# openai/multiagent-particle-envs

Hardware: AMD Instinct MI355X
Metric: env steps/sec (whole node), simple_spread N=3, batch=65536 per GPU (higher is better)
Workload: dtype f32; 1 GPU; simple_spread A=3 L=3, 65536 worlds/GPU, fresh one-hot moves, reset every 25 steps; steps commanded to the step server; protocol=fresh, step-server (one doorbell per episode), batch_per_gpu=65536, global_batch=65536, mode=step-server, commands=auto, barrier_backend=none

## Files before the change

### multiagent_particle_envs_amd/csrc/mpe_split.hip

```cpp
#include <type_traits>

#include "mpe_internal.h"

#ifndef MPE_SPLIT_ABLATE
#define MPE_SPLIT_ABLATE 0
#endif

#ifdef MPE_PHASE_CLOCK
#define MPE_STAMP(k)                                                                                              \
  do {                                                                                                            \
    if (blockIdx.x < 4 && lane == 0 && b.force && t < 32)                                                         \
      reinterpret_cast<unsigned long long *>(b.force)[(((size_t)blockIdx.x * 16 + role) * 32 + t) * 8 + (k)] =     \
          __builtin_amdgcn_s_memtime();                                                                           \
  } while (0)
#else
#define MPE_STAMP(k) do { } while (0)
#endif

#ifdef MPE_DEVICE_SPAN
#define MPE_SPAN_BEGIN() const unsigned long long span_t0_ = (unsigned long long)wall_clock64()
#define MPE_SPAN_END()                                                                                             \
  do {                                                                                                             \
    if (b_in.force && (threadIdx.x & 63) == 0 && (threadIdx.x >> 6) < 8) {                                           \
      const uintptr_t sp_ = reinterpret_cast<uintptr_t>(b_in.force);                                                \
      if (sp_ & 1) asm volatile("s_waitcnt vmcnt(0) lgkmcnt(0)" ::: "memory");                                      \
      ulonglong2 st_;                                                                                              \
      st_.x = span_t0_;                                                                                            \
      st_.y = (unsigned long long)wall_clock64();                                                                  \
      reinterpret_cast<ulonglong2 *>(sp_ & ~(uintptr_t)7)[(size_t)blockIdx.x * 8 + (threadIdx.x >> 6)] = st_;       \
    }                                                                                                              \
  } while (0)
#else
#define MPE_SPAN_BEGIN() do { } while (0)
#define MPE_SPAN_END() do { } while (0)
#endif

namespace mpe {

#ifndef MPE_SPLIT_DUAL
#define MPE_SPLIT_DUAL 1
#endif
#ifndef MPE_SPLIT_DUAL_OWN_DRAW
#define MPE_SPLIT_DUAL_OWN_DRAW (1 << MPE_SCN_SPREAD)
#endif
template <int KIND>
constexpr bool dual_own_draw() { return ((MPE_SPLIT_DUAL_OWN_DRAW) >> KIND) & 1; }

template <int KIND>
constexpr bool dual_kind() {
  return (MPE_SPLIT_DUAL) &&
         (KIND == MPE_SCN_SIMPLE || KIND == MPE_SCN_SPREAD || KIND == MPE_SCN_TAG || KIND == MPE_SCN_ADVERSARY || KIND == MPE_SCN_PUSH);
}

template <int KIND, int A, int L, int NADV>
struct SplitShape {
  static constexpr int E = A + L;
  static constexpr int XW = KIND == MPE_SCN_SPREAD ? 4 + L
                            : (KIND == MPE_SCN_SIMPLE || KIND == MPE_SCN_ADVERSARY || KIND == MPE_SCN_PUSH ||
                               KIND == MPE_SCN_SPEAKER_LISTENER || KIND == MPE_SCN_REFERENCE) ? 5
                            : KIND == MPE_SCN_WORLD_COMM ? 6 : 4;
  static constexpr int DC = KIND == MPE_SCN_SPEAKER_LISTENER ? 3 : KIND == MPE_SCN_REFERENCE ? 10
                            : (KIND == MPE_SCN_CRYPTO || KIND == MPE_SCN_WORLD_COMM) ? 4 : 2;
  static constexpr int NCH = (KIND == MPE_SCN_ADVERSARY || KIND == MPE_SCN_PUSH || KIND == MPE_SCN_SPEAKER_LISTENER) ? 1
                             : (KIND == MPE_SCN_REFERENCE || KIND == MPE_SCN_CRYPTO) ? 2 : 0;
  static constexpr int DMAX = KIND == MPE_SCN_SIMPLE   ? 2 + 2 * L
                              : KIND == MPE_SCN_SPREAD ? 4 + 2 * L + 4 * (A - 1)
                              : KIND == MPE_SCN_TAG    ? 4 + 2 * L + 2 * (A - 1) + 2 * (A - NADV)
                              : KIND == MPE_SCN_ADVERSARY ? 2 + 2 * L + 2 * (A - 1)
                              : KIND == MPE_SCN_PUSH   ? 7 + 5 * L + 2 * (A - 1)
                              : KIND == MPE_SCN_SPEAKER_LISTENER ? 2 + 2 * L + 3
                              : KIND == MPE_SCN_REFERENCE ? 2 + 2 * L + 3 + 10
                              : KIND == MPE_SCN_CRYPTO ? 8
                              : KIND == MPE_SCN_WORLD_COMM ? 4 + 2 * L + 2 * (A - 1) + 2 * (A - NADV) + 2 + 4
// ... 399 lines not shown
};
__device__ __forceinline__ unsigned long long door_load(const unsigned long long *p) {
  const unsigned long long v = __hip_atomic_load(p, __ATOMIC_RELAXED, __HIP_MEMORY_SCOPE_SYSTEM);
  const uint32_t lo = __builtin_amdgcn_readfirstlane((uint32_t)v), hi = __builtin_amdgcn_readfirstlane((uint32_t)(v >> 32));
  return ((unsigned long long)hi << 32) | lo;
}
__device__ __forceinline__ void drain_stores() { asm volatile("s_waitcnt vmcnt(0)" ::: "memory"); }

template <int KIND, int A, int L, int NADV, bool ROLL, int RP ,
          bool DUALP = false ,
          bool SERVE = false ,
          bool POL = false >
__device__ __forceinline__ void split_body(float *const g_pos, float *const g_vel, const float *const g_act, const int32_t *const g_ids,
                                           const size_t B, const int g_wpw, const int g_observe_only, const unsigned g_movable,
                                           const NarrowDesc &d, const MpeBuffers &b_in, const RollArgs &ra, const ServeArgs &sv,
                                           const PolArgs &pol) {
  static_assert(!SERVE || (ROLL && RP == kRowsSc1), "the step server: a rollout instantiation, write-through stores");
  static_assert(!POL || (ROLL && !SERVE && !DUALP), "the policy rollout: a single-role rollout instantiation");
  static_assert(!POL || KIND == MPE_SCN_SIMPLE || KIND == MPE_SCN_SPREAD || KIND == MPE_SCN_ADVERSARY || KIND == MPE_SCN_PUSH,
                "the policy rollout: scenarios whose observation rows read no other agent's velocity");
  constexpr int WM = SERVE ? kWordRowSys : (ROLL ? kWordDrawn : kWordRow);
  using S = SplitShape<KIND, A, L, NADV>;
  MPE_SPAN_BEGIN();
  MpeBuffers b = b_in;
  b.pos = g_pos;
  b.vel = g_vel;
  b.act = g_act;
  b.ids = g_ids;
  constexpr int E = A + L, XW = S::XW;
  constexpr int AUX = SERVE ? kRowsSc1 : aux_policy<KIND, RP>();
  extern __shared__ __attribute__((aligned(16))) float smem[];
  const int lane = threadIdx.x & (kWave - 1);
  constexpr bool DUAL = DUALP && ROLL;
  constexpr bool OWN_DRAW = DUAL && dual_own_draw<KIND>();
  constexpr int NAW = DUAL ? 2 * A : A;
  const int role = __builtin_amdgcn_readfirstlane((int)(threadIdx.x >> 6));
  const bool is_agent = role < NAW;
  const bool is_rows = DUAL && role >= A && role < NAW;
  const int i = is_agent ? (role >= A ? role - A : role) : 0;
  const int wpw = g_wpw;
  const size_t w0 = (size_t)blockIdx.x * (size_t)wpw;
  if (w0 >= B) return;
#ifdef MPE_STRESS_DELAY_WAVE
  if (role == (MPE_STRESS_DELAY_WAVE) % A)
    for (int k = 0; k < 10; ++k) __builtin_amdgcn_s_sleep(127);
#endif
  const int nvalid = (B - w0) < (size_t)wpw ? (int)(B - w0) : wpw;
  const bool live = lane < nvalid;
  const unsigned ln = (unsigned)(live ? lane : nvalid - 1) & 63u;
  const size_t w = w0 + (size_t)ln;
  float *const xch = smem;
  float *const tile = smem + (ROLL ? 2 : 1) * A * XW * kWave + i * S::tile_floats(ROLL);
  int *const mv = reinterpret_cast<int *>(smem + (ROLL ? 2 : 1) * A * XW * kWave + A * S::tile_floats(ROLL));

  const int T = ROLL ? ra.T : 1;
  const size_t obs_stride = (ra.trajectory || SERVE) ? (size_t)d.obs_off[A] * B : 0;
  const size_t row_stride = (ra.trajectory || SERVE) ? (size_t)A * B : 0;
  int blk0 = 0, mvt0 = 0;
  unsigned long long seen = 0;
  int *const idle_cnt = reinterpret_cast<int *>(smem + SplitShape<KIND, A, L, NADV>::lds_bytes(true) / sizeof(float));
  if constexpr (SERVE) {
    blk0 = (int)(ra.step0 % (uint64_t)sv.slots);
    mvt0 = (int)(ra.step0 % (uint64_t)sv.ring);
    if (threadIdx.x < 3) idle_cnt[threadIdx.x] = 0;
    __syncthreads();
  }
// ... 12 lines not shown
    if (seen > g) return true;
    drain_stores();
    bool told = t == 0;
    if (!publisher && !told && lane == 0) __hip_atomic_fetch_add(&idle_cnt[t & 1], 1, __ATOMIC_RELEASE, __HIP_MEMORY_SCOPE_WORKGROUP);
    const unsigned long long t_begin = (unsigned long long)wall_clock64();
    for (;;) {
      if (publisher && !told) {
        const int n = __builtin_amdgcn_readfirstlane(__hip_atomic_load(&idle_cnt[t & 1], __ATOMIC_ACQUIRE, __HIP_MEMORY_SCOPE_WORKGROUP));
        if (n >= NAW) {
          if (lane == 0) __hip_atomic_store(sv.flag + blockIdx.x, g, __ATOMIC_RELAXED, __HIP_MEMORY_SCOPE_SYSTEM);
          told = true;
        }
      }
      __builtin_amdgcn_s_sleep(4);
      seen = door_load(sv.door);
      if (seen > g) return true;
      if ((unsigned long long)wall_clock64() - t_begin > sv.timeout_ticks) {
        if (lane == 0) {
          __hip_atomic_store(sv.status, 1u, __ATOMIC_RELAXED, __HIP_MEMORY_SCOPE_SYSTEM);
          __hip_atomic_store(&idle_cnt[2], 1, __ATOMIC_RELAXED, __HIP_MEMORY_SCOPE_WORKGROUP);
        }
        return false;
      }
    }
  };
  auto next_commanded = [&](const int t) -> bool {
    if constexpr (!SERVE) return false;
    return t + 1 < T && seen > ra.step0 + (unsigned long long)t + 1;
  };
  auto aborted = [&]() -> bool {
    if constexpr (!SERVE) return false;
    return __builtin_amdgcn_readfirstlane(__hip_atomic_load(&idle_cnt[2], __ATOMIC_RELAXED, __HIP_MEMORY_SCOPE_WORKGROUP)) != 0;
  };

  if (!is_agent) {
    constexpr bool TRACK = ROLL && (KIND == MPE_SCN_CRYPTO || KIND == MPE_SCN_WORLD_COMM);
    const uint64_t gw_r = ra.world_offset + w;
    int goal_r = (ROLL && KIND == MPE_SCN_CRYPTO) ? (b.choice + wave_off(w0))[ln] : 0;
    float food[4] = {0.f, 0.f, 0.f, 0.f};
    if (ROLL && KIND == MPE_SCN_WORLD_COMM) {
#pragma unroll
      for (int f = 0; f < 2; ++f) {
        food[2 * f] = (b.pos + wave_off((size_t)(2 * (A + 1 + f)) * B + w0))[ln];
        food[2 * f + 1] = (b.pos + wave_off((size_t)(2 * (A + 1 + f) + 1) * B + w0))[ln];
      }
    }
    float sz[E];
#pragma unroll
    for (int e = 0; e < E; ++e) sz[e] = d.size[e];
    pin_s(sz);
    int cd = -1;
    uint64_t ep_r = 0;
    if (TRACK && ra.episode_len > 0) {
      const uint64_t len = (uint64_t)ra.episode_len, r = ra.step0 % len;
      cd = r == 0 ? 0 : (int)(len - r);
      ep_r = ra.step0 / len + (r ? 1 : 0);
    }
    for (int t = 0; t < T; ++t) {
      MPE_STAMP(0);
      if (SERVE && !wait_door(t, true)) {
        __syncthreads();
        return;
      }
      if (TRACK && cd >= 0) {
        if (cd == 0) {
          if (KIND == MPE_SCN_CRYPTO) goal_r = choice_draw(ra.seed, gw_r, ep_r, 0, d.choice_pop[0]);
          if (KIND == MPE_SCN_WORLD_COMM) {
#pragma unroll
            for (int f = 0; f < 2; ++f) reset_draw(ra.seed, gw_r, ep_r, A + 1 + f, ra.landmark_range, food[2 * f], food[2 * f + 1]);
          }
          ++ep_r;
          cd = ra.episode_len - 1;
        } else {
          --cd;
        }
      }
      if (ROLL && !SERVE && !OWN_DRAW && !POL && t + 1 < T) {
        const uint64_t gt1 = ra.step0 + (uint64_t)t + 1;
#pragma unroll
        for (int q = 0; q < (A + 3) / 4; ++q) {
          const U4 o = action_block(ra.seed, gw_r, gt1, q);
          const uint32_t word[4] = {o.x, o.y, o.z, o.w};
#pragma unroll
          for (int k = 0; k < 4; ++k)
            if (4 * q + k < A) mv[(((t + 1) & 1) * A + 4 * q + k) * kWave + lane] = move_of(word[k]);
        }
      }
      const float *const X = xch + (ROLL ? (t & 1) * A * XW * kWave : 0);
      MPE_STAMP(1);
      if (SERVE) drain_stores();
      __syncthreads();
      if (SERVE) {
        if (t > 0 && lane == 0) __hip_atomic_store(sv.flag + blockIdx.x, ra.step0 + (unsigned long long)t, __ATOMIC_RELAXED, __HIP_MEMORY_SCOPE_SYSTEM);
        if (lane == 0) idle_cnt[t & 1] = 0;
        if (aborted()) return;
      }
      MPE_STAMP(2);
      if (!(MPE_SPLIT_ABLATE & 2))
      reward_wave<KIND, A, L, NADV, ROLL, AUX, WM>(d, sz, with_words(t), X, lane, live, ln, B, w0, (size_t)block_of(t) * row_stride + w0,
                                                   ra.seed, gw_r, ra.step0 + (uint64_t)t, goal_r, food);
      MPE_STAMP(3);
    }
    if (SERVE) {
      drain_stores();
      __syncthreads();
      if (lane == 0) __hip_atomic_store(sv.flag + blockIdx.x, ra.step0 + (unsigned long long)T, __ATOMIC_RELAXED, __HIP_MEMORY_SCOPE_SYSTEM);
    }
    MPE_SPAN_END();
    return;
  }

  float px[E], py[E];
#pragma unroll
  for (int e = 0; e < E; ++e) {
    px[e] = (b.pos + wave_off((size_t)(2 * e) * B + w0))[ln];
    py[e] = (b.pos + wave_off((size_t)(2 * e + 1) * B + w0))[ln];
  }
  float mvx = (b.vel + wave_off((size_t)(2 * i) * B + w0))[ln];
  float mvy = (b.vel + wave_off((size_t)(2 * i + 1) * B + w0))[ln];
  const bool movable_i = (g_movable >> i) & 1u;
  const bool step_world = ROLL || !g_observe_only;
  float ux0 = 0.f, uy0 = 0.f;
  if (!ROLL && step_world && movable_i && (b.act || b.ids)) fetch_action_wave(b, B, i, w0, ln, 1.0f, ux0, uy0);

  float kc[9 + E];
  kc[0] = d.size[i]; kc[1] = d.inv_mass[i]; kc[2] = d.accel[i]; kc[3] = d.max_speed[i];
  kc[4] = d.dt; kc[5] = d.damp; kc[6] = d.cforce; kc[7] = d.cmargin; kc[8] = d.cmargin_inv;
#pragma unroll
// ... 14 lines not shown
  constexpr int NCH = S::NCH, DC = S::DC;
  int goal = NCH >= 1 ? (b.choice + wave_off(w0))[ln] : 0;
  int pick1 = NCH >= 2 ? (b.choice + wave_off(B + w0))[ln] : 0;

  int countdown = -1;
  uint64_t ep = 0;
  if (ROLL && ra.episode_len > 0) {
    const uint64_t len = (uint64_t)ra.episode_len, r = ra.step0 % len;
    countdown = r == 0 ? 0 : (int)(len - r);
    ep = ra.step0 / len + (r ? 1 : 0);
  }

  float gx = 0.f, gy = 0.f;
  [[maybe_unused]] bool did_reset = false;
  auto roll_reset = [&]() -> bool {
    const bool reset_now = countdown == 0;
    if (countdown >= 0) countdown = reset_now ? ra.episode_len - 1 : countdown - 1;
    if (reset_now) {
#pragma unroll
      for (int e = 0; e < E; ++e) reset_draw(ra.seed, gw, ep, e, e < A ? 1.0f : ra.landmark_range, px[e], py[e]);
#pragma unroll
      for (int a = 0; a < A; ++a)
        if (a == i) { mx = px[a]; my = py[a]; }
      mvx = 0.f;
      mvy = 0.f;
      if (NCH >= 1) goal = choice_draw(ra.seed, gw, ep, 0, d.choice_pop[0]);
      if (NCH >= 2) pick1 = choice_draw(ra.seed, gw, ep, 1, d.choice_pop[1]);
      ++ep;
      if (SERVE) did_reset = true;
    }
    return reset_now;
  };
  [[maybe_unused]] float pa1 = 0.f, pa2 = 0.f, pa3 = 0.f, pa4 = 0.f;
  auto step_forces = [&](const int t, float &fx, float &fy) {
    float ux, uy;
    const uint64_t gt = ra.step0 + (uint64_t)t;
    if (ROLL) {
      if constexpr (!POL) roll_reset();
      if constexpr (SERVE) {
        const float *const mt = sv.act_ring + (size_t)((mvt0 + t) % sv.ring) * ((size_t)A * B * MPE_ACTION_DIM);
        typedef float vf4 __attribute__((ext_vector_type(4)));
        const float *const mp = mt + wave_off(((size_t)i * B + w0) * MPE_ACTION_DIM) + (ln * MPE_ACTION_DIM + 1);
        vf4 m4;
        asm volatile("global_load_dwordx4 %0, %1, off sc0 sc1\n\ts_waitcnt vmcnt(0)" : "=&v"(m4) : "v"(mp) : "memory");
        if (movable_i) {
          ux = (m4.x - m4.y) * accel_i;
          uy = (m4.z - m4.w) * accel_i;
        } else {
          ux = 0.f;
          uy = 0.f;
        }
      } else if constexpr (POL) {
        ux = (pa1 - pa2) * accel_i;
        uy = (pa3 - pa4) * accel_i;
      } else {
      const int m = (t == 0 || OWN_DRAW) ? action_draw(ra.seed, gw, gt, i) : mv[((t & 1) * A + i) * kWave + lane];
      ux = ((m == 1 ? 1.f : 0.f) - (m == 2 ? 1.f : 0.f)) * accel_i;
      uy = ((m == 3 ? 1.f : 0.f) - (m == 4 ? 1.f : 0.f)) * accel_i;
      }
    } else if (step_world && movable_i) {
      if (b.act || b.ids) { ux = ux0 * accel_i; uy = uy0 * accel_i; }
      else fetch_action_wave(b, B, i, w0, ln, accel_i, ux, uy);
    } else {
      ux = 0.f;
      uy = 0.f;
    }
    fx = ux + 0.f;
    fy = uy + 0.f;
    if (movable_i && step_world && collide_i && !(MPE_SPLIT_ABLATE & 1)) {
#pragma unroll
      for (int j = 0; j < E; ++j) {
        if (j == i) continue;
        if (!((d.collide >> j) & 1u)) continue;
        float cx, cy;
        contact_force(mx - px[j], my - py[j], size_i + size_e[j], k_cforce, k_cmargin, k_cmargin_inv, cx, cy);
        fx = cx + fx;
        fy = cy + fy;
// ... 7 lines not shown
      if (live && (!ROLL || t == T - 1)) store_state<AUX>(b, B, i, w0, ln, mx, my, mvx, mvy);
#endif
    }
#ifdef MPE_PHASE_CLOCK
    asm volatile("" ::"v"(mx), "v"(my), "v"(mvx), "v"(mvy));
#endif
  };
  auto publish = [&](const int t) {
    float *const X = xch + (ROLL ? (t & 1) * A * XW * kWave : 0);
    X[(i * XW + 0) * kWave + lane] = mx;
    X[(i * XW + 1) * kWave + lane] = my;
    X[(i * XW + 2) * kWave + lane] = mvx;
    X[(i * XW + 3) * kWave + lane] = mvy;
    if (KIND == MPE_SCN_SPREAD) {
#pragma unroll
      for (int l = 0; l < L; ++l) X[(i * XW + 4 + l) * kWave + lane] = sq2d(mx - px[A + l], my - py[A + l]);
    }
    if (KIND == MPE_SCN_SIMPLE) X[(i * XW + 4) * kWave + lane] = sq2d(mx - px[A], my - py[A]);
    if (HAS_GOAL || KIND == MPE_SCN_SPEAKER_LISTENER) {
      goal_pos<A, L>(px, py, goal, gx, gy);
      X[(i * XW + 4) * kWave + lane] = sq2d(mx - gx, my - gy);
    }
    if constexpr (KIND == MPE_SCN_REFERENCE) {
      goal_pos<A, L>(px, py, i == 0 ? pick1 : goal, gx, gy);
      X[(i * XW + 4) * kWave + lane] = sq2d(mx - gx, my - gy);
    }
    if constexpr (KIND == MPE_SCN_WORLD_COMM) {
#pragma unroll
      for (int f = 0; f < 2; ++f)
        X[(i * XW + 4 + f) * kWave + lane] =
            sqrt_lt(sq2d(mx - px[A + 3 + f], my - py[A + 3 + f]), size_i + size_e[A + 3 + f]) ? 1.f : -1.f;
    }
  };
  auto behind_barrier = [&](const int t) {
#ifndef MPE_STRESS_STORE_BEFORE_BARRIER
    if (movable_i && step_world && live && (!ROLL || (SERVE ? !next_commanded(t) : t == T - 1)) && !(MPE_SPLIT_ABLATE & 8))
      store_state<AUX>(b, B, i, w0, ln, mx, my, mvx, mvy);
#endif
    if constexpr (SERVE) {
      if (did_reset && live) {
#pragma unroll
        for (int l = 0; l < L; ++l)
          if (l % A == i) {
            store_aux<AUX>(b.pos + wave_off((size_t)(2 * (A + l)) * B + w0) + ln, px[A + l]);
            store_aux<AUX>(b.pos + wave_off((size_t)(2 * (A + l) + 1) * B + w0) + ln, py[A + l]);
          }
        if (NCH >= 1 && i == 0) {
          store_aux<AUX>(b.choice + wave_off(w0) + ln, goal);
          if (NCH >= 2) store_aux<AUX>(b.choice + wave_off(B + w0) + ln, pick1);
        }
        if (!movable_i) store_state<AUX>(b, B, i, w0, ln, mx, my, mvx, mvy);
      }
      did_reset = false;
    }
    if constexpr (KIND == MPE_SCN_ADVERSARY && !ROLL) {
      if (live && b.info_rew) {
        store_aux<AUX>(b.info_rew + wave_off((size_t)i * B + w0) + ln, sq2d(mx - gx, my - gy));
        if (b.info_min_dists) {
#pragma unroll
          for (int l = 0; l < L; ++l)
            store_aux<AUX>(b.info_min_dists + wave_off(((size_t)l * A + i) * B + w0) + ln, sq2d(mx - px[A + l], my - py[A + l]));
        }
      }
    }
    const float *const X = xch + (ROLL ? (t & 1) * A * XW * kWave : 0);
#pragma unroll
    for (int a = 0; a < A; ++a) {
      if (a == i) { px[a] = mx; py[a] = my; continue; }
      px[a] = X[(a * XW + 0) * kWave + lane];
      py[a] = X[(a * XW + 1) * kWave + lane];
    }
#ifdef MPE_PHASE_CLOCK
#pragma unroll
    for (int a = 0; a < A; ++a) asm volatile("" ::"v"(px[a]), "v"(py[a]));
#endif
  };
  [[maybe_unused]] int pol_D = 0, pol_S = 0, pol_sw = 0;
  auto note_tile = [&](auto dc, auto pc) {
    if constexpr (POL) {
      constexpr int D = decltype(dc)::value;
      constexpr bool P = decltype(pc)::value;
      constexpr int NS = (P && row_vec4<D>()) ? D / 4 : 0;
      pol_D = D;
      pol_S = P ? pair_stride<D>() : tile_stride<D>();
      pol_sw = NS ? swz4<NS>(lane) : 0;
    }
  };
  auto rows = [&](const int t, const bool pre) {
    if (MPE_SPLIT_ABLATE & 4) return;
    const float *const X = xch + (ROLL ? (t & 1) * A * XW * kWave : 0);
    const uint64_t gt = ra.step0 + (uint64_t)t;
    float *const obs_t = b.obs + (size_t)block_of(t) * obs_stride;
    [[maybe_unused]] const MpeBuffers bw = with_words(t);
    if (KIND == MPE_SCN_SIMPLE) {
      constexpr int D = 2 + 2 * L;
      {
        RowPairs<D> r(tile, lane);
        r.put(0, mvx, mvy);
#pragma unroll
        for (int l = 0; l < L; ++l) r.put(2 + 2 * l, px[A + l] - mx, py[A + l] - my);
      }
      note_tile(std::integral_constant<int, D>{}, std::bool_constant<true>{});
        if (!pre) flush_rows<D, true, RP>(tile, obs_t + B * obs_off_i + w0 * D, nvalid, lane, d.vec4);
    }
    if (KIND == MPE_SCN_SPREAD) {
      constexpr int D = 4 + 2 * L + 4 * (A - 1);
      {
        RowPairs<D> r(tile, lane);
        r.put(0, mvx, mvy);
        r.put(2, mx, my);
#pragma unroll
        for (int l = 0; l < L; ++l) r.put(4 + 2 * l, px[A + l] - mx, py[A + l] - my);
        int k = 4 + 2 * L;
#pragma unroll
        for (int j = 0; j < A; ++j) {
          if (j == i) continue;
          r.put(k, px[j] - mx, py[j] - my);
          k += 2;
        }
#pragma unroll
        for (int z = 0; z < 2 * (A - 1); z += 2) r.put(k + z, 0.f, 0.f);
      }
      note_tile(std::integral_constant<int, D>{}, std::bool_constant<true>{});
        if (!pre) flush_rows<D, true, RP>(tile, obs_t + B * obs_off_i + w0 * D, nvalid, lane, d.vec4);
    }
    if (KIND == MPE_SCN_TAG) {
      constexpr int NG = A - NADV;
      constexpr int DA = 4 + 2 * L + 2 * (A - 1) + 2 * NG, DG = DA - 2;
      const bool adv = i < NADV;
      auto row = [&](auto dsel) {
        constexpr int D = decltype(dsel)::value;
        {
          RowPairs<D> r(tile, lane);
          r.put(0, mvx, mvy);
          r.put(2, mx, my);
#pragma unroll
          for (int l = 0; l < L; ++l) r.put(4 + 2 * l, px[A + l] - mx, py[A + l] - my);
          int k = 4 + 2 * L;
#pragma unroll
          for (int j = 0; j < A; ++j) {
            if (j == i) continue;
            r.put(k, px[j] - mx, py[j] - my);
            k += 2;
          }
#pragma unroll
          for (int j = NADV; j < A; ++j) {
            if (j == i) continue;
            r.put(k, X[(j * XW + 2) * kWave + lane], X[(j * XW + 3) * kWave + lane]);
            k += 2;
          }
        }
        note_tile(std::integral_constant<int, D>{}, std::bool_constant<true>{});
        if (!pre) flush_rows<D, true, RP>(tile, obs_t + B * obs_off_i + w0 * D, nvalid, lane, d.vec4);
      };
      if (adv) row(std::integral_constant<int, DA>{});
      else     row(std::integral_constant<int, DG>{});
    }
    if (KIND == MPE_SCN_ADVERSARY) {
      constexpr int DG = 2 + 2 * L + 2 * (A - 1), DA = DG - 2;
      const bool adv = i < NADV;
      auto row = [&](auto dsel, auto good) {
        constexpr int D = decltype(dsel)::value;
        {
          RowPairs<D> r(tile, lane);
          int k = 0;
          if (decltype(good)::value) { r.put(k, gx - mx, gy - my); k += 2; }
#pragma unroll
          for (int l = 0; l < L; ++l) { r.put(k, px[A + l] - mx, py[A + l] - my); k += 2; }
#pragma unroll
          for (int j = 0; j < A; ++j) {
            if (j == i) continue;
            r.put(k, px[j] - mx, py[j] - my);
            k += 2;
          }
        }
        note_tile(std::integral_constant<int, D>{}, std::bool_constant<true>{});
        if (!pre) flush_rows<D, true, RP>(tile, obs_t + B * obs_off_i + w0 * D, nvalid, lane, d.vec4);
      };
      if (adv) row(std::integral_constant<int, DA>{}, std::false_type{});
      else     row(std::integral_constant<int, DG>{}, std::true_type{});
    }
    if constexpr (KIND == MPE_SCN_PUSH) {
      constexpr int DG = 7 + 5 * L + 2 * (A - 1), DA = 2 + 2 * L + 2 * (A - 1);
      const bool adv = i < NADV;
      auto row = [&](auto dsel, auto good) {
        constexpr int D = decltype(dsel)::value, RS = tile_stride<D>();
        constexpr bool GOOD = decltype(good)::value;
        int k = 0;
        if (GOOD || (RS & 1)) { put1<RS>(tile, lane, k, mvx); put1<RS>(tile, lane, k + 1, mvy); }
        else put2<RS>(tile, lane, k, mvx, mvy);
        k += 2;
        if (GOOD) {
          put1<RS>(tile, lane, k, gx - mx); put1<RS>(tile, lane, k + 1, gy - my);
          k += 2;
#pragma unroll
          for (int c = 0; c < 3; ++c) put1<RS>(tile, lane, k + c, (goal + 1 == c) ? 0.75f : 0.25f);
          k += 3;
        }
#pragma unroll
        for (int l = 0; l < L; ++l) {
          if ((RS & 1) || (k & 1)) { put1<RS>(tile, lane, k, px[A + l] - mx); put1<RS>(tile, lane, k + 1, py[A + l] - my); }
          else put2<RS>(tile, lane, k, px[A + l] - mx, py[A + l] - my);
          k += 2;
        }
        if (GOOD) {
#pragma unroll
          for (int l = 0; l < L; ++l)
#pragma unroll
            for (int c = 0; c < 3; ++c) put1<RS>(tile, lane, k + 3 * l + c, (l + 1 == c) ? (float)(0.1 + 0.8) : 0.1f);
          k += 3 * L;
        }
#pragma unroll
        for (int j = 0; j < A; ++j) {
          if (j == i) continue;
          if ((RS & 1) || (k & 1)) { put1<RS>(tile, lane, k, px[j] - mx); put1<RS>(tile, lane, k + 1, py[j] - my); }
          else put2<RS>(tile, lane, k, px[j] - mx, py[j] - my);
          k += 2;
        }
        note_tile(std::integral_constant<int, D>{}, std::bool_constant<false>{});
        if (!pre) flush_rows<D, false, RP>(tile, obs_t + B * obs_off_i + w0 * D, nvalid, lane, d.vec4);
      };
      if (adv) row(std::integral_constant<int, DA>{}, std::false_type{});
      else     row(std::integral_constant<int, DG>{}, std::true_type{});
    }
    if constexpr (KIND == MPE_SCN_SPEAKER_LISTENER) {
      if (i == 0) {
        constexpr int D = 3, RS = tile_stride<D>();
#pragma unroll
        for (int c = 0; c < 3; ++c) put1<RS>(tile, lane, c, goal == c ? 0.65f : 0.15f);
        note_tile(std::integral_constant<int, D>{}, std::bool_constant<false>{});
        if (!pre) flush_rows<D, false, RP>(tile, obs_t + B * obs_off_i + w0 * D, nvalid, lane, d.vec4);
      } else {
        constexpr int D = 2 + 2 * L + DC, RS = tile_stride<D>();
        put1<RS>(tile, lane, 0, mvx); put1<RS>(tile, lane, 1, mvy);
#pragma unroll
        for (int l = 0; l < L; ++l) { put1<RS>(tile, lane, 2 + 2 * l, px[A + l] - mx); put1<RS>(tile, lane, 3 + 2 * l, py[A + l] - my); }
        const Word<WM> c0 = word_of<DC, WM>(bw, B, w0, ln, 0, ra.seed, gw, gt);
#pragma unroll
        for (int c = 0; c < DC; ++c) put1<RS>(tile, lane, 2 + 2 * L + c, c0[c]);
        note_tile(std::integral_constant<int, D>{}, std::bool_constant<false>{});
        if (!pre) flush_rows<D, false, RP>(tile, obs_t + B * obs_off_i + w0 * D, nvalid, lane, d.vec4);
      }
    }
    if constexpr (KIND == MPE_SCN_REFERENCE) {
      constexpr int D = 2 + 2 * L + 3 + DC, RS = tile_stride<D>();
      const int mine = i == 0 ? goal : pick1;
      put1<RS>(tile, lane, 0, mvx); put1<RS>(tile, lane, 1, mvy);
#pragma unroll
      for (int l = 0; l < L; ++l) { put1<RS>(tile, lane, 2 + 2 * l, px[A + l] - mx); put1<RS>(tile, lane, 3 + 2 * l, py[A + l] - my); }
#pragma unroll
      for (int c = 0; c < 3; ++c) put1<RS>(tile, lane, 2 + 2 * L + c, mine == c ? 0.75f : 0.25f);
      const Word<WM> co = word_of<DC, WM>(bw, B, w0, ln, 1 - i, ra.seed, gw, gt);
#pragma unroll
      for (int c = 0; c < DC; ++c) put1<RS>(tile, lane, 5 + 2 * L + c, co[c]);
      note_tile(std::integral_constant<int, D>{}, std::bool_constant<false>{});
        if (!pre) flush_rows<D, false, RP>(tile, obs_t + B * obs_off_i + w0 * D, nvalid, lane, d.vec4);
    }
    if constexpr (KIND == MPE_SCN_CRYPTO) {
      const Word<WM> cs = word_of<DC, WM>(bw, B, w0, ln, 2, ra.seed, gw, gt);
      static_assert((DC & 1) == 0, "crypto rows are written as pairs");
      if (i == 0) {
        constexpr int D = DC;
        RowPairs<D> r(tile, lane);
#pragma unroll
        for (int c = 0; c < DC; c += 2) r.put(c, cs[c], cs[c + 1]);
        note_tile(std::integral_constant<int, D>{}, std::bool_constant<true>{});
        if (!pre) flush_rows<D, true, RP>(tile, obs_t + B * obs_off_i + w0 * D, nvalid, lane, d.vec4);
      } else {
        constexpr int D = 2 * DC;
        RowPairs<D> r(tile, lane);
        const int first = i == 1 ? pick1 : goal;
#pragma unroll
        for (int c = 0; c < DC; c += 2) r.put(c, first == c ? 1.f : 0.f, first == c + 1 ? 1.f : 0.f);
#pragma unroll
        for (int c = 0; c < DC; c += 2) {
          if (i == 1) r.put(DC + c, cs[c], cs[c + 1]);
          else        r.put(DC + c, pick1 == c ? 1.f : 0.f, pick1 == c + 1 ? 1.f : 0.f);
        }
        note_tile(std::integral_constant<int, D>{}, std::bool_constant<true>{});
        if (!pre) flush_rows<D, true, RP>(tile, obs_t + B * obs_off_i + w0 * D, nvalid, lane, d.vec4);
      }
    }
    if constexpr (KIND == MPE_SCN_WORLD_COMM) {
      constexpr int NG = A - NADV;
      constexpr int DA = 4 + 2 * L + 2 * (A - 1) + 2 * NG + 2 + DC, DGd = 4 + 2 * L + 2 * (A - 1) + 2 + 2 * (NG - 1);
      const bool f1 = X[(i * XW + 4) * kWave + lane] > 0.f, f2 = X[(i * XW + 5) * kWave + lane] > 0.f;
      bool vis[A];
#pragma unroll
      for (int j = 0; j < A; ++j) {
        const bool o1 = X[(j * XW + 4) * kWave + lane] > 0.f, o2 = X[(j * XW + 5) * kWave + lane] > 0.f;
        vis[j] = i == 0 || (f1 && o1) || (f2 && o2) || (!f1 && !o1 && !f2 && !o2);
      }
      auto row = [&](auto dsel, auto advt) {
        constexpr int D = decltype(dsel)::value, RS = tile_stride<D>();
        constexpr bool ADV = decltype(advt)::value;
        constexpr bool HALF = S::trows(ROLL) == 32;
#pragma unroll
        for (int h = 0; h < (HALF ? 2 : 1); ++h) {
        const int r = HALF ? (lane & 31) : lane;
        if (!HALF || (lane >> 5) == h) {
        int k = 0;
        put1<RS>(tile, r, 0, mvx); put1<RS>(tile, r, 1, mvy); put1<RS>(tile, r, 2, mx); put1<RS>(tile, r, 3, my);
        k = 4;
#pragma unroll
        for (int l = 0; l < L; ++l) { put1<RS>(tile, r, k, px[A + l] - mx); put1<RS>(tile, r, k + 1, py[A + l] - my); k += 2; }
#pragma unroll
        for (int j = 0; j < A; ++j) {
          if (j == i) continue;
          put1<RS>(tile, r, k, vis[j] ? px[j] - mx : 0.f);
          put1<RS>(tile, r, k + 1, vis[j] ? py[j] - my : 0.f);
          k += 2;
        }
        if (!ADV) { put1<RS>(tile, r, k, f1 ? 1.f : -1.f); put1<RS>(tile, r, k + 1, f2 ? 1.f : -1.f); k += 2; }
#pragma unroll
        for (int j = NADV; j < A; ++j) {
          if (j == i) continue;
          put1<RS>(tile, r, k, vis[j] ? X[(j * XW + 2) * kWave + lane] : 0.f);
          put1<RS>(tile, r, k + 1, vis[j] ? X[(j * XW + 3) * kWave + lane] : 0.f);
          k += 2;
        }
        if (ADV) {
          put1<RS>(tile, r, k, f1 ? 1.f : -1.f); put1<RS>(tile, r, k + 1, f2 ? 1.f : -1.f); k += 2;
          const Word<WM> cl = word_of<DC, WM>(bw, B, w0, ln, 0, ra.seed, gw, gt);
#pragma unroll
          for (int c = 0; c < DC; ++c) put1<RS>(tile, r, k + c, cl[c]);
        }
        }
        const int nv = HALF ? min(max(nvalid - 32 * h, 0), 32) : nvalid;
        if (nv > 0) flush_rows<D, false, RP>(tile, obs_t + B * obs_off_i + (w0 + (HALF ? 32 * h : 0)) * D, nv, lane, d.vec4);
        }
      };
      if (i < NADV) row(std::integral_constant<int, DA>{}, std::true_type{});
      else          row(std::integral_constant<int, DGd>{}, std::false_type{});
    }
  };
  [[maybe_unused]] auto decide = [&](const int t) {
    const uint64_t gt = ra.step0 + (uint64_t)t;
    const bool rs = roll_reset();
    if (t == 0 || rs) {
      if (HAS_GOAL) goal_pos<A, L>(px, py, goal, gx, gy);
      rows(t, true);
    }
    float *const rec = (pol.obs_in && live) ? pol.obs_in + wave_off((size_t)t * (size_t)d.obs_off[A] * B + B * (size_t)obs_off_i + w0 * (size_t)pol_D) +
                                                  ln * pol_D
                                            : nullptr;
    float z[5];
    pol_logits(pol.w + pol.off[i], pol.nl[i], pol.act[i] != 0, tile + lane * pol_S, pol_sw, pol_D, rec, z);
    float zm = z[0];
    int am = 0;
#pragma unroll
    for (int j = 1; j < 5; ++j)
      if (z[j] > zm) { zm = z[j]; am = j; }
    float e[5], sum = 0.f;
#pragma unroll
    for (int j = 0; j < 5; ++j) {
      e[j] = __expf(z[j] - zm);
      sum += e[j];
    }
    float r[5];
    int m = am;
    if (pol.mode == MPE_POLICY_SOFTMAX) {
#pragma unroll
      for (int j = 0; j < 5; ++j) r[j] = e[j] / sum;
    } else {
      if (pol.mode == MPE_POLICY_SAMPLE) {
        const float u = (float)(policy_bits(pol.seed, gw, gt, i) >> 8) * (1.0f / 16777216.0f);
        float c = 0.f;
        m = 4;
        float cj[4];
#pragma unroll
        for (int j = 0; j < 4; ++j) {
          c += e[j] / sum;
          cj[j] = c;
        }
// ... 24 lines not shown
    if (is_rows) {
      for (int t = 0; t < T; ++t) {
        MPE_STAMP(0);
        const bool reset_now = countdown == 0;
        if (countdown >= 0) countdown = reset_now ? ra.episode_len - 1 : countdown - 1;
        if (reset_now) {
#pragma unroll
          for (int l = 0; l < L; ++l) reset_draw(ra.seed, gw, ep, A + l, ra.landmark_range, px[A + l], py[A + l]);
          if (NCH >= 1) goal = choice_draw(ra.seed, gw, ep, 0, d.choice_pop[0]);
          if (NCH >= 2) pick1 = choice_draw(ra.seed, gw, ep, 1, d.choice_pop[1]);
          ++ep;
        }
        if (HAS_GOAL || KIND == MPE_SCN_SPEAKER_LISTENER) goal_pos<A, L>(px, py, goal, gx, gy);
        MPE_STAMP(2);
        __syncthreads();
        if (SERVE && aborted()) return;
        MPE_STAMP(3);
        const float *const X = xch + (t & 1) * A * XW * kWave;
        mx = X[(i * XW + 0) * kWave + lane];
        my = X[(i * XW + 1) * kWave + lane];
        mvx = X[(i * XW + 2) * kWave + lane];
        mvy = X[(i * XW + 3) * kWave + lane];
#pragma unroll
        for (int a = 0; a < A; ++a) {
          if (a == i) { px[a] = mx; py[a] = my; continue; }
          px[a] = X[(a * XW + 0) * kWave + lane];
          py[a] = X[(a * XW + 1) * kWave + lane];
        }
#ifdef MPE_PHASE_CLOCK
#pragma unroll
        for (int a = 0; a < A; ++a) asm volatile("" ::"v"(px[a]), "v"(py[a]));
#endif
        MPE_STAMP(4);
        rows(t, false);
        MPE_STAMP(5);
        if constexpr (SERVE) {
          drain_stores();
          if (lane == 0) __hip_atomic_fetch_add(&idle_cnt[(t + 1) & 1], 1, __ATOMIC_RELEASE, __HIP_MEMORY_SCOPE_WORKGROUP);
        }
      }
      if (SERVE) __syncthreads();
      MPE_SPAN_END();
      return;
    }
    float fx, fy;
    { [[maybe_unused]] const int t = 0; MPE_STAMP(0); }
    if (SERVE && !wait_door(0, false)) {
      __syncthreads();
      return;
    }
    step_forces(0, fx, fy);
    step_integrate(0, fx, fy);
    { [[maybe_unused]] const int t = 0; MPE_STAMP(1); }
    publish(0);
    for (int t = 0; t < T; ++t) {
      MPE_STAMP(2);
      if (SERVE) drain_stores();
      __syncthreads();
      if (SERVE && aborted()) return;
      MPE_STAMP(3);
      behind_barrier(t);
      MPE_STAMP(4);
      if (t + 1 < T) {
        if (SERVE && !wait_door(t + 1, false)) {
          __syncthreads();
          return;
        }
        step_forces(t + 1, fx, fy);
        step_integrate(t + 1, fx, fy);
        MPE_STAMP(5);
        publish(t + 1);
      }
    }
    if (SERVE) {
      drain_stores();
      __syncthreads();
      MPE_SPAN_END();
      return;
    }
  } else {
    for (int t = 0; t < T; ++t) {
      float fx, fy;
      MPE_STAMP(0);
      if (SERVE && !wait_door(t, false)) {
        __syncthreads();
        return;
      }
      if constexpr (POL) decide(t);
      step_forces(t, fx, fy);
      step_integrate(t, fx, fy);
      MPE_STAMP(1);
      publish(t);
      MPE_STAMP(2);
      if (SERVE) drain_stores();
      __syncthreads();
      if (SERVE && aborted()) return;
      MPE_STAMP(3);
      behind_barrier(t);
      MPE_STAMP(4);
      rows(t, false);
      MPE_STAMP(5);
    }
    if (SERVE) {
      drain_stores();
      __syncthreads();
      MPE_SPAN_END();
      return;
    }
  }
  if (ROLL && NCH >= 1 && ra.episode_len > 0 && live && i == 0) {
    store_aux<AUX>(b.choice + wave_off(w0) + ln, goal);
    if (NCH >= 2) store_aux<AUX>(b.choice + wave_off(B + w0) + ln, pick1);
  }
  if (ROLL && ((speakers_of<KIND>() >> i) & 1u) && live && T > 0) {
    float *const mine = const_cast<float *>(b.comm) + wave_off(((size_t)i * B + w0) * DC) + ln * DC;
    const int id = comm_draw(ra.seed, gw, ra.step0 + (uint64_t)(T - 1), i, DC);
#pragma unroll
    for (int c = 0; c < DC; ++c) mine[c] = c == id ? 1.f : 0.f;
  }
  if (ROLL && ra.episode_len > 0 && live) {
#pragma unroll
    for (int l = 0; l < L; ++l)
      if (l % A == i) {
        (b.pos + wave_off((size_t)(2 * (A + l)) * B + w0))[ln] = px[A + l];
        (b.pos + wave_off((size_t)(2 * (A + l) + 1) * B + w0))[ln] = py[A + l];
      }
    if (!movable_i) {
      store_aux<AUX>(b.pos + wave_off((size_t)(2 * i) * B + w0) + ln, mx);
      store_aux<AUX>(b.pos + wave_off((size_t)(2 * i + 1) * B + w0) + ln, my);
      store_aux<AUX>(b.vel + wave_off((size_t)(2 * i) * B + w0) + ln, mvx);
      store_aux<AUX>(b.vel + wave_off((size_t)(2 * i + 1) * B + w0) + ln, mvy);
    }
  }
  MPE_SPAN_END();
// ... 145 lines not shown
  if (e->lds > 64 * 1024) {
    const hipError_t rc = hipFuncSetAttribute(reinterpret_cast<const void *>(e->fn), hipFuncAttributeMaxDynamicSharedMemorySize, (int)e->lds);
    if (rc != hipSuccess) return (int)rc;
  }
  hipLaunchKernelGGL(e->fn, dim3(grid), dim3((A + 1) * kWave), e->lds, stream, b.pos, b.vel, b.act, b.ids, B, (int)r2.wpw, 0,
                     (unsigned)d.movable, d, b, r2, pol);
  return (int)hipGetLastError();
}

bool serve_supports(int kind, int A, int L, int nadv) {
  const SplitEntry *e = find_split(kind, A, L, nadv);
  return e && e->serve;
}
unsigned serve_grid(size_t B) { return (unsigned)((B + kWave - 1) / kWave); }

int launch_split_serve(int kind, int A, int L, int nadv, const NarrowDesc &d, const MpeBuffers &b, size_t B, const RollArgs &ra,
                       const ServeHandles &h, hipStream_t stream) {
  const SplitEntry *e = find_split(kind, A, L, nadv);
  if (!e || !e->serve) return MPE_EUNSUPPORTED;
  RollArgs r2 = ra;
  r2.wpw = kWave;
  ServeArgs sv;
  sv.door = reinterpret_cast<unsigned long long *>(h.door);
  sv.flag = reinterpret_cast<unsigned long long *>(h.flag);
  sv.status = h.status;
  sv.act_ring = h.act_ring;
  sv.comm_ring = h.comm_ring;
  sv.ring = h.ring;
  sv.slots = h.slots;
  sv.timeout_ticks = h.timeout_ticks;
  const size_t lds = e->lds_roll + 16;
  const unsigned grid = serve_grid(B);
  int per_cu = 0, dev = 0, n_cu = 0;
  if (hipGetDevice(&dev) != hipSuccess || hipDeviceGetAttribute(&n_cu, hipDeviceAttributeMultiprocessorCount, dev) != hipSuccess) {
    (void)hipGetLastError();
    return MPE_EUNSUPPORTED;
  }
  SplitFn fn = e->serve;
  int waves = A + 1;
#ifndef MPE_SERVE_NO_DUAL
  if (e->serve_dual && grid <= (unsigned)n_cu * 3 / 2) {
    fn = e->serve_dual;
    waves = 2 * A + 1;
  }
#endif
  if (hipOccupancyMaxActiveBlocksPerMultiprocessor(&per_cu, reinterpret_cast<const void *>(fn), waves * kWave, lds) != hipSuccess) {
    (void)hipGetLastError();
    return MPE_EUNSUPPORTED;
  }
  if (!h.ahead && (size_t)grid > (size_t)n_cu * (size_t)(per_cu > 1 ? per_cu - 1 : per_cu)) return MPE_ESERVER_TOO_LARGE;
  hipLaunchKernelGGL(fn, dim3(grid), dim3(waves * kWave), lds, stream, b.pos, b.vel, b.act, b.ids, B, (int)r2.wpw, 0,
                     (unsigned)d.movable, d, b, r2, sv);
  return (int)hipGetLastError();
}

__global__ void k_serve_ring(unsigned long long *const door, const unsigned long long n) {
  if (threadIdx.x == 0 && blockIdx.x == 0) __hip_atomic_fetch_add(door, n, __ATOMIC_RELAXED, __HIP_MEMORY_SCOPE_SYSTEM);
}
__global__ void __launch_bounds__(256)
k_serve_wait(const unsigned long long *const flag, const unsigned n_flags, const unsigned long long completed,
             unsigned int *const status, const unsigned long long timeout_ticks) {
  const unsigned k = blockIdx.x * blockDim.x + threadIdx.x;
  if (k >= n_flags) return;
  const unsigned long long t0 = (unsigned long long)wall_clock64();
  while (__hip_atomic_load(flag + k, __ATOMIC_RELAXED, __HIP_MEMORY_SCOPE_SYSTEM) < completed) {
    __builtin_amdgcn_s_sleep(8);
    if ((unsigned long long)wall_clock64() - t0 > timeout_ticks) {
      __hip_atomic_store(status, 2u, __ATOMIC_RELAXED, __HIP_MEMORY_SCOPE_SYSTEM);
      return;
    }
  }
}
int launch_serve_ring(uint64_t *door, uint64_t n, hipStream_t stream) {
  hipLaunchKernelGGL(k_serve_ring, dim3(1), dim3(64), 0, stream, reinterpret_cast<unsigned long long *>(door), (unsigned long long)n);
  return (int)hipGetLastError();
}
int launch_serve_wait(const uint64_t *flag, unsigned n_flags, uint64_t completed, uint32_t *status, uint64_t timeout_ticks,
                      hipStream_t stream) {
  hipLaunchKernelGGL(k_serve_wait, dim3((n_flags + 255) / 256), dim3(256), 0, stream, reinterpret_cast<const unsigned long long *>(flag),
                     n_flags, (unsigned long long)completed, status, (unsigned long long)timeout_ticks);
  return (int)hipGetLastError();
}

// ... 2 lines not shown
```

Measured before the change: 19.26 billion env-steps/s.

## Pipeline next-step move loads across the server step barrier

In the step-server kernel, when the next step is already commanded, agent waves issue the next step's action-ring load before the store and row phase and skip the per-step doorbell wait and store drain. The non-agent wave publishes a pipelined flag per step and holds the completion flag back by one step. This is meant to hide the action-load latency and the barrier and drain round trips between consecutive commanded steps. Separately, the host launcher caches the CU count and occupancy query per device and kernel, cutting per-launch API overhead. The cost is more complex synchronisation, with risks around flag ordering and store visibility.

```diff
diff --git a/multiagent_particle_envs_amd/csrc/mpe_split.hip b/multiagent_particle_envs_amd/csrc/mpe_split.hip
--- a/multiagent_particle_envs_amd/csrc/mpe_split.hip
+++ b/multiagent_particle_envs_amd/csrc/mpe_split.hip
@@ -1,4 +1,7 @@
+#include <map>
+#include <mutex>
 #include <type_traits>
+#include <utility>
 
 #include "mpe_internal.h"
 
@@ -39,6 +42,9 @@
 
 #ifndef MPE_SPLIT_DUAL
 #define MPE_SPLIT_DUAL 1
+#endif
+#ifndef MPE_SERVE_PIPE_SINGLE
+#define MPE_SERVE_PIPE_SINGLE 0
 #endif
 #ifndef MPE_SPLIT_DUAL_OWN_DRAW
 #define MPE_SPLIT_DUAL_OWN_DRAW (1 << MPE_SCN_SPREAD)
@@ -504,6 +510,7 @@
   extern __shared__ __attribute__((aligned(16))) float smem[];
   const int lane = threadIdx.x & (kWave - 1);
   constexpr bool DUAL = DUALP && ROLL;
+  constexpr bool PIPE = SERVE && (DUALP || (MPE_SERVE_PIPE_SINGLE));
   constexpr bool OWN_DRAW = DUAL && dual_own_draw<KIND>();
   constexpr int NAW = DUAL ? 2 * A : A;
   const int role = __builtin_amdgcn_readfirstlane((int)(threadIdx.x >> 6));
@@ -582,6 +589,39 @@
     if constexpr (!SERVE) return false;
     return __builtin_amdgcn_readfirstlane(__hip_atomic_load(&idle_cnt[2], __ATOMIC_RELAXED, __HIP_MEMORY_SCOPE_WORKGROUP)) != 0;
   };
+  int *const pipe = mv;
+  auto pipelined = [&](const int t) -> bool {
+    if constexpr (!PIPE) return false;
+    return __builtin_amdgcn_readfirstlane(__hip_atomic_load(&pipe[t & 1], __ATOMIC_RELAXED, __HIP_MEMORY_SCOPE_WORKGROUP)) != 0;
+  };
+  typedef float vf4 __attribute__((ext_vector_type(4)));
+  auto move_issue = [&](const int t) -> vf4 {
+    const float *const mt = sv.act_ring + (size_t)((mvt0 + t) % sv.ring) * ((size_t)A * B * MPE_ACTION_DIM);
+    const float *const mp = mt + wave_off(((size_t)i * B + w0) * MPE_ACTION_DIM) + (ln * MPE_ACTION_DIM + 1);
+    vf4 raw;
+    asm volatile("global_load_dwordx4 %0, %1, off sc0 sc1" : "=&v"(raw) : "v"(mp) : "memory");
+    return raw;
+  };
+  auto move_wait = [&](const vf4 raw) -> vf4 {
+    vf4 m4;
+    asm volatile("s_waitcnt vmcnt(0)\n\tv_mov_b32 %0, %4\n\tv_mov_b32 %1, %5\n\tv_mov_b32 %2, %6\n\tv_mov_b32 %3, %7"
+                 : "=&v"(m4.x), "=&v"(m4.y), "=&v"(m4.z), "=&v"(m4.w)
+                 : "v"(raw.x), "v"(raw.y), "v"(raw.z), "v"(raw.w)
+                 : "memory");
+    return m4;
+  };
+  [[maybe_unused]] vf4 m4_next = {0.f, 0.f, 0.f, 0.f}, m4_raw = {0.f, 0.f, 0.f, 0.f};
+  [[maybe_unused]] bool flush_wait = false;
+  auto before_flush = [&](auto piped) {
+    if constexpr (SERVE) {
+      if constexpr (decltype(piped)::value) {
+        m4_next = move_wait(m4_raw);
+      } else if (flush_wait) {
+        drain_stores();
+        flush_wait = false;
+      }
+    }
+  };
 
   if (!is_agent) {
     constexpr bool TRACK = ROLL && (KIND == MPE_SCN_CRYPTO || KIND == MPE_SCN_WORLD_COMM);
@@ -606,6 +646,7 @@
       cd = r == 0 ? 0 : (int)(len - r);
       ep_r = ra.step0 / len + (r ? 1 : 0);
     }
+    [[maybe_unused]] bool prev_pip = false;
     for (int t = 0; t < T; ++t) {
       MPE_STAMP(0);
       if (SERVE && !wait_door(t, true)) {
@@ -638,12 +679,19 @@
       }
       const float *const X = xch + (ROLL ? (t & 1) * A * XW * kWave : 0);
       MPE_STAMP(1);
-      if (SERVE) drain_stores();
+      [[maybe_unused]] const bool pip = PIPE && next_commanded(t);
+      if (SERVE) {
+        drain_stores();
+        if (PIPE && lane == 0) __hip_atomic_store(&pipe[t & 1], pip ? 1 : 0, __ATOMIC_RELAXED, __HIP_MEMORY_SCOPE_WORKGROUP);
+      }
       __syncthreads();
       if (SERVE) {
-        if (t > 0 && lane == 0) __hip_atomic_store(sv.flag + blockIdx.x, ra.step0 + (unsigned long long)t, __ATOMIC_RELAXED, __HIP_MEMORY_SCOPE_SYSTEM);
+        const int done = t - (prev_pip ? 1 : 0);
+        if (done > 0 && lane == 0)
+          __hip_atomic_store(sv.flag + blockIdx.x, ra.step0 + (unsigned long long)done, __ATOMIC_RELAXED, __HIP_MEMORY_SCOPE_SYSTEM);
         if (lane == 0) idle_cnt[t & 1] = 0;
         if (aborted()) return;
+        prev_pip = pip;
       }
       MPE_STAMP(2);
       if (!(MPE_SPLIT_ABLATE & 2))
@@ -724,17 +772,16 @@
     return reset_now;
   };
   [[maybe_unused]] float pa1 = 0.f, pa2 = 0.f, pa3 = 0.f, pa4 = 0.f;
-  auto step_forces = [&](const int t, float &fx, float &fy) {
+  auto step_forces = [&](const int t, float &fx, float &fy, [[maybe_unused]] const bool have_move = false) {
     float ux, uy;
     const uint64_t gt = ra.step0 + (uint64_t)t;
     if (ROLL) {
       if constexpr (!POL) roll_reset();
       if constexpr (SERVE) {
-        const float *const mt = sv.act_ring + (size_t)((mvt0 + t) % sv.ring) * ((size_t)A * B * MPE_ACTION_DIM);
-        typedef float vf4 __attribute__((ext_vector_type(4)));
-        const float *const mp = mt + wave_off(((size_t)i * B + w0) * MPE_ACTION_DIM) + (ln * MPE_ACTION_DIM + 1);
-        vf4 m4;
-        asm volatile("global_load_dwordx4 %0, %1, off sc0 sc1\n\ts_waitcnt vmcnt(0)" : "=&v"(m4) : "v"(mp) : "memory");
+        vf4 m4 = m4_next;
+        if (!have_move) {
+          m4 = move_wait(move_issue(t));
+        }
         if (movable_i) {
           ux = (m4.x - m4.y) * accel_i;
           uy = (m4.z - m4.w) * accel_i;
@@ -808,9 +855,9 @@
             sqrt_lt(sq2d(mx - px[A + 3 + f], my - py[A + 3 + f]), size_i + size_e[A + 3 + f]) ? 1.f : -1.f;
     }
   };
-  auto behind_barrier = [&](const int t) {
+  auto behind_barrier = [&](const int t, [[maybe_unused]] const bool at_rest = true) {
 #ifndef MPE_STRESS_STORE_BEFORE_BARRIER
-    if (movable_i && step_world && live && (!ROLL || (SERVE ? !next_commanded(t) : t == T - 1)) && !(MPE_SPLIT_ABLATE & 8))
+    if (movable_i && step_world && live && (!ROLL || (SERVE ? (PIPE ? at_rest : !next_commanded(t)) : t == T - 1)) && !(MPE_SPLIT_ABLATE & 8))
       store_state<AUX>(b, B, i, w0, ln, mx, my, mvx, mvy);
 #endif
     if constexpr (SERVE) {
@@ -862,8 +909,17 @@
       pol_sw = NS ? swz4<NS>(lane) : 0;
     }
   };
-  auto rows = [&](const int t, const bool pre) {
-    if (MPE_SPLIT_ABLATE & 4) return;
+  auto early_wait = [&](auto piped) {
+    if constexpr (decltype(piped)::value) before_flush(piped);
+  };
+  auto late_wait = [&](auto piped) {
+    if constexpr (!decltype(piped)::value) before_flush(piped);
+  };
+  auto rows = [&](const int t, const bool pre, [[maybe_unused]] auto piped) {
+    if (MPE_SPLIT_ABLATE & 4) {
+      before_flush(piped);
+      return;
+    }
     const float *const X = xch + (ROLL ? (t & 1) * A * XW * kWave : 0);
     const uint64_t gt = ra.step0 + (uint64_t)t;
     float *const obs_t = b.obs + (size_t)block_of(t) * obs_stride;
@@ -877,6 +933,7 @@
         for (int l = 0; l < L; ++l) r.put(2 + 2 * l, px[A + l] - mx, py[A + l] - my);
       }
       note_tile(std::integral_constant<int, D>{}, std::bool_constant<true>{});
+        before_flush(piped);
         if (!pre) flush_rows<D, true, RP>(tile, obs_t + B * obs_off_i + w0 * D, nvalid, lane, d.vec4);
     }
     if (KIND == MPE_SCN_SPREAD) {
@@ -898,9 +955,11 @@
         for (int z = 0; z < 2 * (A - 1); z += 2) r.put(k + z, 0.f, 0.f);
       }
       note_tile(std::integral_constant<int, D>{}, std::bool_constant<true>{});
+        before_flush(piped);
         if (!pre) flush_rows<D, true, RP>(tile, obs_t + B * obs_off_i + w0 * D, nvalid, lane, d.vec4);
     }
     if (KIND == MPE_SCN_TAG) {
+      early_wait(piped);
       constexpr int NG = A - NADV;
       constexpr int DA = 4 + 2 * L + 2 * (A - 1) + 2 * NG, DG = DA - 2;
       const bool adv = i < NADV;
@@ -927,12 +986,14 @@
           }
         }
         note_tile(std::integral_constant<int, D>{}, std::bool_constant<true>{});
+        late_wait(piped);
         if (!pre) flush_rows<D, true, RP>(tile, obs_t + B * obs_off_i + w0 * D, nvalid, lane, d.vec4);
       };
       if (adv) row(std::integral_constant<int, DA>{});
       else     row(std::integral_constant<int, DG>{});
     }
     if (KIND == MPE_SCN_ADVERSARY) {
+      early_wait(piped);
       constexpr int DG = 2 + 2 * L + 2 * (A - 1), DA = DG - 2;
       const bool adv = i < NADV;
       auto row = [&](auto dsel, auto good) {
@@ -951,12 +1012,14 @@
           }
         }
         note_tile(std::integral_constant<int, D>{}, std::bool_constant<true>{});
+        late_wait(piped);
         if (!pre) flush_rows<D, true, RP>(tile, obs_t + B * obs_off_i + w0 * D, nvalid, lane, d.vec4);
       };
       if (adv) row(std::integral_constant<int, DA>{}, std::false_type{});
       else     row(std::integral_constant<int, DG>{}, std::true_type{});
     }
     if constexpr (KIND == MPE_SCN_PUSH) {
+      early_wait(piped);
       constexpr int DG = 7 + 5 * L + 2 * (A - 1), DA = 2 + 2 * L + 2 * (A - 1);
       const bool adv = i < NADV;
       auto row = [&](auto dsel, auto good) {
@@ -994,17 +1057,20 @@
           k += 2;
         }
         note_tile(std::integral_constant<int, D>{}, std::bool_constant<false>{});
+        late_wait(piped);
         if (!pre) flush_rows<D, false, RP>(tile, obs_t + B * obs_off_i + w0 * D, nvalid, lane, d.vec4);
       };
       if (adv) row(std::integral_constant<int, DA>{}, std::false_type{});
       else     row(std::integral_constant<int, DG>{}, std::true_type{});
     }
     if constexpr (KIND == MPE_SCN_SPEAKER_LISTENER) {
+      early_wait(piped);
       if (i == 0) {
         constexpr int D = 3, RS = tile_stride<D>();
 #pragma unroll
         for (int c = 0; c < 3; ++c) put1<RS>(tile, lane, c, goal == c ? 0.65f : 0.15f);
         note_tile(std::integral_constant<int, D>{}, std::bool_constant<false>{});
+        late_wait(piped);
         if (!pre) flush_rows<D, false, RP>(tile, obs_t + B * obs_off_i + w0 * D, nvalid, lane, d.vec4);
       } else {
         constexpr int D = 2 + 2 * L + DC, RS = tile_stride<D>();
@@ -1015,6 +1081,7 @@
 #pragma unroll
         for (int c = 0; c < DC; ++c) put1<RS>(tile, lane, 2 + 2 * L + c, c0[c]);
         note_tile(std::integral_constant<int, D>{}, std::bool_constant<false>{});
+        late_wait(piped);
         if (!pre) flush_rows<D, false, RP>(tile, obs_t + B * obs_off_i + w0 * D, nvalid, lane, d.vec4);
       }
     }
@@ -1030,9 +1097,11 @@
 #pragma unroll
       for (int c = 0; c < DC; ++c) put1<RS>(tile, lane, 5 + 2 * L + c, co[c]);
       note_tile(std::integral_constant<int, D>{}, std::bool_constant<false>{});
+        before_flush(piped);
         if (!pre) flush_rows<D, false, RP>(tile, obs_t + B * obs_off_i + w0 * D, nvalid, lane, d.vec4);
     }
     if constexpr (KIND == MPE_SCN_CRYPTO) {
+      early_wait(piped);
       const Word<WM> cs = word_of<DC, WM>(bw, B, w0, ln, 2, ra.seed, gw, gt);
       static_assert((DC & 1) == 0, "crypto rows are written as pairs");
       if (i == 0) {
@@ -1041,6 +1110,7 @@
 #pragma unroll
         for (int c = 0; c < DC; c += 2) r.put(c, cs[c], cs[c + 1]);
         note_tile(std::integral_constant<int, D>{}, std::bool_constant<true>{});
+        late_wait(piped);
         if (!pre) flush_rows<D, true, RP>(tile, obs_t + B * obs_off_i + w0 * D, nvalid, lane, d.vec4);
       } else {
         constexpr int D = 2 * DC;
@@ -1054,10 +1124,12 @@
           else        r.put(DC + c, pick1 == c ? 1.f : 0.f, pick1 == c + 1 ? 1.f : 0.f);
         }
         note_tile(std::integral_constant<int, D>{}, std::bool_constant<true>{});
+        late_wait(piped);
         if (!pre) flush_rows<D, true, RP>(tile, obs_t + B * obs_off_i + w0 * D, nvalid, lane, d.vec4);
       }
     }
     if constexpr (KIND == MPE_SCN_WORLD_COMM) {
+      early_wait(piped);
       constexpr int NG = A - NADV;
       constexpr int DA = 4 + 2 * L + 2 * (A - 1) + 2 * NG + 2 + DC, DGd = 4 + 2 * L + 2 * (A - 1) + 2 + 2 * (NG - 1);
       const bool f1 = X[(i * XW + 4) * kWave + lane] > 0.f, f2 = X[(i * XW + 5) * kWave + lane] > 0.f;
@@ -1103,6 +1175,7 @@
         }
         }
         const int nv = HALF ? min(max(nvalid - 32 * h, 0), 32) : nvalid;
+        if (h == 0) late_wait(piped);
         if (nv > 0) flush_rows<D, false, RP>(tile, obs_t + B * obs_off_i + (w0 + (HALF ? 32 * h : 0)) * D, nv, lane, d.vec4);
         }
       };
@@ -1115,7 +1188,7 @@
     const bool rs = roll_reset();
     if (t == 0 || rs) {
       if (HAS_GOAL) goal_pos<A, L>(px, py, goal, gx, gy);
-      rows(t, true);
+      rows(t, true, std::false_type{});
     }
     float *const rec = (pol.obs_in && live) ? pol.obs_in + wave_off((size_t)t * (size_t)d.obs_off[A] * B + B * (size_t)obs_off_i + w0 * (size_t)pol_D) +
                                                   ln * pol_D
@@ -1206,11 +1279,15 @@
         for (int a = 0; a < A; ++a) asm volatile("" ::"v"(px[a]), "v"(py[a]));
 #endif
         MPE_STAMP(4);
-        rows(t, false);
+        [[maybe_unused]] const bool pip = pipelined(t);
+        flush_wait = pip;
+        rows(t, false, std::false_type{});
         MPE_STAMP(5);
         if constexpr (SERVE) {
-          drain_stores();
-          if (lane == 0) __hip_atomic_fetch_add(&idle_cnt[(t + 1) & 1], 1, __ATOMIC_RELEASE, __HIP_MEMORY_SCOPE_WORKGROUP);
+          if (!pip) {
+            drain_stores();
+            if (lane == 0) __hip_atomic_fetch_add(&idle_cnt[(t + 1) & 1], 1, __ATOMIC_RELEASE, __HIP_MEMORY_SCOPE_WORKGROUP);
+          }
         }
       }
       if (SERVE) __syncthreads();
@@ -1233,14 +1310,21 @@
       __syncthreads();
       if (SERVE && aborted()) return;
       MPE_STAMP(3);
-      behind_barrier(t);
+      [[maybe_unused]] const bool pip = pipelined(t);
+      if (SERVE && pip) {
+        m4_raw = move_issue(t + 1);
+        behind_barrier(t, false);
+        m4_next = move_wait(m4_raw);
+      } else {
+        behind_barrier(t);
+      }
       MPE_STAMP(4);
       if (t + 1 < T) {
-        if (SERVE && !wait_door(t + 1, false)) {
+        if (SERVE && !pip && !wait_door(t + 1, false)) {
           __syncthreads();
           return;
         }
-        step_forces(t + 1, fx, fy);
+        step_forces(t + 1, fx, fy, pip);
         step_integrate(t + 1, fx, fy);
         MPE_STAMP(5);
         publish(t + 1);
@@ -1253,27 +1337,37 @@
       return;
     }
   } else {
+    [[maybe_unused]] bool prev_pip = false;
     for (int t = 0; t < T; ++t) {
       float fx, fy;
       MPE_STAMP(0);
-      if (SERVE && !wait_door(t, false)) {
+      if (SERVE && !prev_pip && !wait_door(t, false)) {
         __syncthreads();
         return;
       }
       if constexpr (POL) decide(t);
-      step_forces(t, fx, fy);
+      step_forces(t, fx, fy, prev_pip);
       step_integrate(t, fx, fy);
       MPE_STAMP(1);
       publish(t);
       MPE_STAMP(2);
-      if (SERVE) drain_stores();
+      if (SERVE && !prev_pip) drain_stores();
       __syncthreads();
       if (SERVE && aborted()) return;
       MPE_STAMP(3);
-      behind_barrier(t);
-      MPE_STAMP(4);
-      rows(t, false);
+      [[maybe_unused]] const bool pip = pipelined(t);
+      if (SERVE && pip) {
+        m4_raw = move_issue(t + 1);
+        behind_barrier(t, false);
+        MPE_STAMP(4);
+        rows(t, false, std::true_type{});
+      } else {
+        behind_barrier(t);
+        MPE_STAMP(4);
+        rows(t, false, std::false_type{});
+      }
       MPE_STAMP(5);
+      prev_pip = pip;
     }
     if (SERVE) {
       drain_stores();
@@ -1485,9 +1579,25 @@
   const size_t lds = e->lds_roll + 16;
   const unsigned grid = serve_grid(B);
   int per_cu = 0, dev = 0, n_cu = 0;
-  if (hipGetDevice(&dev) != hipSuccess || hipDeviceGetAttribute(&n_cu, hipDeviceAttributeMultiprocessorCount, dev) != hipSuccess) {
+  if (hipGetDevice(&dev) != hipSuccess) {
     (void)hipGetLastError();
     return MPE_EUNSUPPORTED;
+  }
+  static std::mutex cache_mu;
+  static std::map<int, int> cu_of;
+  static std::map<std::pair<int, const void *>, int> per_cu_of;
+  {
+    std::lock_guard<std::mutex> lk(cache_mu);
+    const auto it = cu_of.find(dev);
+    if (it != cu_of.end()) n_cu = it->second;
+  }
+  if (n_cu == 0) {
+    if (hipDeviceGetAttribute(&n_cu, hipDeviceAttributeMultiprocessorCount, dev) != hipSuccess || n_cu <= 0) {
+      (void)hipGetLastError();
+      return MPE_EUNSUPPORTED;
+    }
+    std::lock_guard<std::mutex> lk(cache_mu);
+    cu_of[dev] = n_cu;
   }
   SplitFn fn = e->serve;
   int waves = A + 1;
@@ -1497,11 +1607,25 @@
     waves = 2 * A + 1;
   }
 #endif
-  if (hipOccupancyMaxActiveBlocksPerMultiprocessor(&per_cu, reinterpret_cast<const void *>(fn), waves * kWave, lds) != hipSuccess) {
-    (void)hipGetLastError();
-    return MPE_EUNSUPPORTED;
-  }
-  if (!h.ahead && (size_t)grid > (size_t)n_cu * (size_t)(per_cu > 1 ? per_cu - 1 : per_cu)) return MPE_ESERVER_TOO_LARGE;
+  if (!h.ahead) {
+    const std::pair<int, const void *> key(dev, reinterpret_cast<const void *>(fn));
+    {
+      std::lock_guard<std::mutex> lk(cache_mu);
+      const auto it = per_cu_of.find(key);
+      if (it != per_cu_of.end()) per_cu = it->second;
+    }
+    if (per_cu == 0) {
+      if (hipOccupancyMaxActiveBlocksPerMultiprocessor(&per_cu, reinterpret_cast<const void *>(fn), waves * kWave, lds) != hipSuccess) {
+        (void)hipGetLastError();
+        return MPE_EUNSUPPORTED;
+      }
+      if (per_cu > 0) {
+        std::lock_guard<std::mutex> lk(cache_mu);
+        per_cu_of[key] = per_cu;
+      }
+    }
+    if ((size_t)grid > (size_t)n_cu * (size_t)(per_cu > 1 ? per_cu - 1 : per_cu)) return MPE_ESERVER_TOO_LARGE;
+  }
   hipLaunchKernelGGL(fn, dim3(grid), dim3(waves * kWave), lds, stream, b.pos, b.vel, b.act, b.ids, B, (int)r2.wpw, 0,
                      (unsigned)d.movable, d, b, r2, sv);
   return (int)hipGetLastError();
```

New measurement: 19.03 billion env-steps/s. 1.2% lower.
